# Chlumsky/msdfgen

Hardware: AMD Instinct MI355X
Metric: MSDF glyphs/sec (64x64, fp32) (higher is better)
Workload: dtype f64

## Files before the change

### msdfgen_amd/csrc/msdf_capi.hip

```cpp

#include <hip/hip_runtime.h>

#include <algorithm>
#include <atomic>
#include <chrono>
#include <condition_variable>
#include <cmath>
#include <cstdarg>
#include <cstdio>
#include <cstdlib>
#include <cstring>
#include <deque>
#include <functional>
#include <memory>
#include <mutex>
#include <string>
#include <thread>
#include <vector>

#include <sched.h>

#include "msdf_classplan.hpp"
#include "msdf_hostplan.hpp"
#include "msdf_kernels.hpp"
// ... 881 lines not shown
        return rc;
    ScopedTimer timer(stream, 1, !paramsOnly);
    if (cfg.ec_stage_limit != 0) {
        if (paramsOnly)
            return MSDFHIP_OK;
        const unsigned cap = GRES ? slowGrid : 16384u;
        const unsigned slowBlocks = (unsigned) ((allTexels+WAVE-1)/WAVE < cap ? (allTexels+WAVE-1)/WAVE : cap);
        hipLaunchKernelGGL((k_ec_slow<N, OVERLAP, GRES>), dim3(slowBlocks), dim3(WAVE), slowLds, stream, viewOf(b), dGlyphs, w, h, src, out, stencil, cfg,
                           (const EcCandidate *) NULL, 0u, 0, gres, gresStride);
        HIPCHK(hipGetLastError());
        return MSDFHIP_OK;
    }
    const unsigned seg = ecSegment((size_t) w*h);
    const size_t cap = deferredRecords(b->nGlyphs, (size_t) w*h, b->nEdges);
    EcCandidate *deferred = NULL;
    rc = ensureDeferred(b, cap, &deferred);
    if (rc != MSDFHIP_OK)
        return rc;
    const int slotCapWanted = tuning().querySlotCap, lpcContoursWanted = tuning().queryLpcContours;
    int slotCap = b->maxEdges < slotCapWanted ? (b->maxEdges > 0 ? b->maxEdges : 1) : slotCapWanted;
    bool wideSlots = false;
    if (b->nGlyphs < 256 && !tuning().hasQueryLds) {
        const int wide = b->maxEdges < 1024 ? (b->maxEdges > 0 ? b->maxEdges : 1) : 1024;
        const int wideMerged = b->maxContours < wide ? (b->maxContours > 0 ? b->maxContours : 1) : wide;
        if ((size_t) b->maxContours*sizeof(double)+(size_t) (wide+wideMerged)*sizeof(PBSlot) <= (size_t) 64*1024 && wide > slotCap)
            slotCap = wide, wideSlots = true;
    }
    EcQueryPolicy lpcMaxContours;
    lpcMaxContours.lpcMaxContours = b->maxContours < lpcContoursWanted ? b->maxContours : lpcContoursWanted;
    lpcMaxContours.lpcEdgeCost = tuning().qpEdgeCost, lpcMaxContours.lpcMaxEdges = tuning().qpMaxEdges, lpcMaxContours.lpcMinCount = tuning().qpMinCount;
    lpcMaxContours.wideMaxEdges = tuning().qpWideMaxEdges, lpcMaxContours.wideLoad = tuning().qpWideLoad, lpcMaxContours.wideMeanCount = tuning().qpWideMeanCount;
    lpcMaxContours.gridSteps = tuning().queryGridSteps;
    const size_t resLanes = OVERLAP ? (size_t) (lpcMaxContours.lpcMaxContours > 0 ? lpcMaxContours.lpcMaxContours : 1)*WAVE*sizeof(double) : 0;
    const int slotOffset = OVERLAP ? (b->maxContours > 0 ? b->maxContours : 1) : 0;
    const int mergedCap = b->maxContours < slotCap ? (b->maxContours > 0 ? b->maxContours : 1) : slotCap;
    const size_t coopLds = (size_t) slotOffset*sizeof(double)+(size_t) (slotCap+mergedCap)*sizeof(PBSlot);
    const size_t queryLds = resLanes > coopLds ? resLanes : coopLds;
    const size_t fastLds = ecFastLdsBytes(b->maxEdges, N);
    if (GRES && queryLds > (size_t) gLdsLimit.load() && fastLds <= (size_t) gLdsLimit.load()) {
        if (paramsOnly)
            return MSDFHIP_OK;
        hipLaunchKernelGGL((k_ec_slow<N, OVERLAP, GRES>), dim3(slowGrid), dim3(WAVE), slowLds, stream, viewOf(b), dGlyphs, w, h, src, out, stencil, cfg,
                           (const EcCandidate *) NULL, 0u, 0, gres, gresStride);
        HIPCHK(hipGetLastError());
        countRoute(MSDFHIP_ROUTE_EC_SLOW_ALL);
        return MSDFHIP_OK;
    }
    if (fastLds > (size_t) gLdsLimit.load() || queryLds > (size_t) gLdsLimit.load())
        return fail(MSDFHIP_ERR_TOO_COMPLEX, "a glyph has %d contours / %d edges: the error-correction pass needs %zu B of LDS per wavefront, device limit is %d B",
                    b->maxContours, b->maxEdges, fastLds > queryLds ? fastLds : queryLds, gLdsLimit.load());
    rc = setLds(k_ec_query<N, OVERLAP>, queryLds);
    if (rc != MSDFHIP_OK)
        return rc;
    rc = setLds(k_ec_fast<N>, fastLds);
    if (rc != MSDFHIP_OK)
        return rc;
    int *offsets = reinterpret_cast<int *>(deferred+candidateRecords(b->nGlyphs, (size_t) w*h));
    int *corners = reinterpret_cast<int *>(deferred+candidateRecords(b->nGlyphs, (size_t) w*h)+offsetRecords(b->nGlyphs));
    const size_t wanted = allTexels/512;
    unsigned queryBlocks = (unsigned) (wanted < 64 ? 64 : wanted > 8192 ? 8192 : wanted);
    const bool staticDeal = tuning().queryStatic != 0;
    if (staticDeal) {
        const unsigned resident = queryResidentBlocks<N, OVERLAP>(b->device, queryLds);
        if (resident && queryBlocks > resident)
            queryBlocks = resident;
    }
    if (!call.ecParamsQueued)
        hipLaunchKernelGGL(k_ec_params, dim3((unsigned) b->nGlyphs), dim3(WAVE), 0, stream, b->work.ecParams.ptr, viewOf(b), dGlyphs, cfg,
                           reinterpret_cast<unsigned *>(deferred), corners, offsets+ecSizesAt(b->nGlyphs));
    const int *ecOrder = NULL;
    rc = ensureEcOrder(b, &ecOrder, stream);
    if (rc != MSDFHIP_OK)
        return rc;
    if (paramsOnly) {
        HIPCHK(hipGetLastError());
        call.ecParamsQueued = true;
        return MSDFHIP_OK;
    }
    hipLaunchKernelGGL((k_ec_fast<N>), dim3(blocks), dim3(WAVE), fastLds, stream, viewOf(b), dGlyphs, w, h, tilesX, tiles, src, out, stencil, cfg,
                       (const EcGlyphParams *) b->work.ecParams.ptr, deferred, seg, b->maxEdges, (const int *) corners);
    hipLaunchKernelGGL(k_ec_scan, dim3(1), dim3(1024), 0, stream, b->nGlyphs, reinterpret_cast<const unsigned *>(deferred), seg, offsets, lpcMaxContours, ecOrder);
    hipLaunchKernelGGL((k_ec_query<N, OVERLAP>), dim3(queryBlocks), dim3(WAVE), queryLds, stream, b->nGlyphs, b->dGlyphContourOffsets, b->dContourOffsets,
                       (const EdgeRec *) viewOf(b).recs, viewOf(b).windings, dGlyphs, w, h, src, out, stencil, cfg,
                       (const EcGlyphParams *) b->work.ecParams.ptr, (const EcCandidate *) deferred, seg, (const int *) offsets, offsets+2*(size_t) b->nGlyphs+2, tuning().queryBatch, slotCap, slotOffset, lpcMaxContours,
                       call.overflowOut, ecOrder, staticDeal ? (tuning().queryStatic == 2 ? 5 : 1) : 0);
    if (call.overflowOut)
        call.overflowMirrored = true;
    else
        hipLaunchKernelGGL((k_ec_slow<N, OVERLAP, GRES>), dim3(slowGrid), dim3(WAVE), slowLds, stream, viewOf(b), dGlyphs, w, h, src, out, stencil, cfg,
                           (const EcCandidate *) deferred, seg, 1, gres, gresStride);
    HIPCHK(hipGetLastError());
    countRoute(ecOrder ? MSDFHIP_ROUTE_EC_QUERY_HEAVIEST : MSDFHIP_ROUTE_EC_QUERY_BATCH);
    if (wideSlots)
        countRoute(MSDFHIP_ROUTE_EC_WIDE_SLOTS);
    return MSDFHIP_OK;
}

template <int N>
int dispatchEc(const MsdfHipBatch *b, const MsdfHipGlyph *dGlyphs, int w, int h, const float *src, float *out, uint8_t *stencil,
               const MsdfHipConfig &cfg, hipStream_t stream, GenerateCall &call, bool paramsOnly) {
    if (!cfg.overlap_support)
        return launchEc<N, false, false>(b, dGlyphs, w, h, src, out, stencil, cfg, stream, call, paramsOnly);
    const bool globalRes = (size_t) b->maxContours*WAVE*sizeof(double) > 96*1024;
    return globalRes ? launchEc<N, true, true>(b, dGlyphs, w, h, src, out, stencil, cfg, stream, call, paramsOnly)
                     : launchEc<N, true, false>(b, dGlyphs, w, h, src, out, stencil, cfg, stream, call, paramsOnly);
}

int checkConfig(const MsdfHipConfig *cfg) {
    if (!cfg)
        return fail(MSDFHIP_ERR_INVALID, "cfg is NULL");
    if (cfg->ec_mode < 0 || cfg->ec_mode > 3 || cfg->ec_distance_check < 0 || cfg->ec_distance_check > 2 || cfg->ec_stage_limit < 0 || cfg->ec_stage_limit > 4)
        return fail(MSDFHIP_ERR_INVALID, "bad error-correction config (mode %d, distance check %d, stage limit %d)", cfg->ec_mode, cfg->ec_distance_check, cfg->ec_stage_limit);
    return MSDFHIP_OK;
}

int ensureScratch(const MsdfHipBatch *b, size_t floats, float **out) {
    std::lock_guard<std::mutex> lock(b->work.mutex);
    HIPCHK(b->work.scratch.ensure(floats));
    *out = b->work.scratch.ptr;
    return MSDFHIP_OK;
}

int runCorrection(const MsdfHipBatch *b, int channels, int w, int h, const MsdfHipGlyph *dGlyphs, const float *src, float *out, uint8_t *stencil,
                  const MsdfHipConfig &cfg, hipStream_t stream, GenerateCall &call, bool paramsOnly) {
    return channels == 3 ? dispatchEc<3>(b, dGlyphs, w, h, src, out, stencil, cfg, stream, call, paramsOnly)
                         : dispatchEc<4>(b, dGlyphs, w, h, src, out, stencil, cfg, stream, call, paramsOnly);
}

int prepareAhead(const MsdfHipBatch *b, int mode, int w, int h, const MsdfHipGlyph *dGlyphs, const MsdfHipConfig *cfg, hipStream_t stream, GenerateCall &call) {
    if (b->nGlyphs == 0 || w == 0 || h == 0)
        return MSDFHIP_OK;
    const int nch = channelsOf(mode);
    const LaunchShape shape = launchShape(b, w, h, nch, false);
// ... 2970 lines not shown
```

### msdfgen_amd/csrc/msdf_ec_fast.hpp

```cpp
#pragma once

#include "msdf_ec.hpp"

namespace msdfhip {

enum { EC_DEFER = 0x80 };

MSDF_HD bool ecHasBasePass(const EcParams &p) { return p.distanceCheck == EC_DO_NOT_CHECK || (p.distanceCheck == EC_CHECK_AT_EDGE && p.mode != EC_MODE_EDGE_ONLY); }
MSDF_HD bool ecHasShapePass(const EcParams &p) { return p.distanceCheck == EC_ALWAYS_CHECK || p.distanceCheck == EC_CHECK_AT_EDGE; }

struct FastCtx {
    double span;
    bool p1;
    bool pShape;
    bool basePass, shapePass;
};

MSDF_HD int rangeTest2(const FastCtx &c, double at, double bt, double xt, float am, float bm, float xm) {
    const bool inversion = (am > .5f && bm > .5f && xm <= .5f) || (am < .5f && bm < .5f && xm >= .5f);
    const bool outside = medianf(am, bm, xm) != xm;
    const bool candBase = c.basePass && (inversion || (!c.p1 && outside));
    const bool candShape = c.shapePass && (inversion || (!c.pShape && outside));
    if (!(candBase || candShape))
        return 0;
    const double axSpan = (xt-at)*c.span, bxSpan = (bt-xt)*c.span;
    const int f = (xm >= am-axSpan && xm <= am+axSpan && xm >= bm-bxSpan && xm <= bm+bxSpan) ? 1 : 3;
    return (candBase ? f : 0)|(candShape ? f<<2 : 0);
}

MSDF_HD int judge(int flags) {
    if (flags&2)
        return 1;
    const int fs = flags>>2;
    if (fs&1)
        return (fs&2) ? 1 : 2;
    return 0;
}

MSDF_HD bool quadraticMayHaveRootInRange(double a, double b, double c) {
    if (a == 0 || fabs(b) > 1e12*fabs(a))
        return true;
    const double lo = .005, hi = .995;
    const double mag = fabs(a)+fabs(b)+fabs(c);
    const double eps = 1e-9*mag;
    const double flo = (a*lo+b)*lo+c, fhi = (a*hi+b)*hi+c;
    if (!(flo > eps && fhi > eps) && !(flo < -eps && fhi < -eps))
        return true;
    const double s = flo > 0 ? 1. : -1.;
    const double as = a*s, bs = b*s, cs = c*s;
    if (as <= 0)
        return false;
    if (!(-bs > 2*as*lo*(1-1e-9) && -bs < 2*as*hi*(1+1e-9)))
        return false;
    return !(4*as*cs-bs*bs > 1e-9*mag*mag);
}

MSDF_HD bool bernsteinMayHaveRoot(float dA, float dBC, float dD) {
    const float m = fmaxf(fmaxf(fabsf(dA), fabsf(dBC)), fabsf(dD));
    const float eps = 1e-5f*m;
    const float h = .5f*dBC;
    return !((dA > eps && h > eps && dD > eps) || (dA < -eps && h < -eps && dD < -eps));
}

MSDF_HD bool edgeBetweenTexelsChannelFast(const float *a, const float *b, int channel) {
    const double n = a[channel]-.5;
    const double d = a[channel]-b[channel];
    if (!((n > 0 && d > 0 && n < d) || (n < 0 && d < 0 && n > d)))
        return false;
    const double t = n/d;
    if (t > 0 && t < 1) {
        float c[3] = { mixf(a[0], b[0], t), mixf(a[1], b[1], t), mixf(a[2], b[2], t) };
        return medianf(c[0], c[1], c[2]) == c[channel];
    }
    return false;
}

MSDF_HD int edgeBetweenTexelsFast(const float *a, const float *b) {
    return 1*(int) edgeBetweenTexelsChannelFast(a, b, 0)+2*(int) edgeBetweenTexelsChannelFast(a, b, 1)+4*(int) edgeBetweenTexelsChannelFast(a, b, 2);
}

template <class Sink>
MSDF_HD int diagonalPairFast(const FastCtx &cx, float am, float dm, const float *a, const float *l, const float *q,
                             float dA, float dBC, float dD, float l0, float q0, float l1, float q1, Sink &sink) {
    const double qa = dD-dBC+dA, qb = dBC-dA-dA, qc = dA;
    if (!quadraticMayHaveRootInRange(qa, qb, qc))
        return 0;
    double t[2];
    const int solutions = solveQuadratic(t, qa, qb, qc);
    int verdict = 0;
    for (int i = 0; i < solutions; ++i) {
        if (t[i] > MSDF_ARTIFACT_T_EPSILON && t[i] < 1-MSDF_ARTIFACT_T_EPSILON) {
            const float xm = interpolatedMedianQuad(a, l, q, t[i]);
            int rangeFlags = rangeTest2(cx, 0, 1, t[i], am, dm, xm);
            const double tEx0 = -.5*l0/q0, tEx1 = -.5*l1/q1;
            if (tEx0 > 0 && tEx0 < 1) {
                double tEnd0 = 0, tEnd1 = 1;
                float em0 = am, em1 = dm;
                const float ex = interpolatedMedianQuad(a, l, q, tEx0);
                if (tEx0 > t[i])
                    tEnd1 = tEx0, em1 = ex;
                else
                    tEnd0 = tEx0, em0 = ex;
                rangeFlags |= rangeTest2(cx, tEnd0, tEnd1, t[i], em0, em1, xm);
            }
            if (tEx1 > 0 && tEx1 < 1) {
                double tEnd0 = 0, tEnd1 = 1;
                float em0 = am, em1 = dm;
                const float ex = interpolatedMedianQuad(a, l, q, tEx1);
                if (tEx1 > t[i])
                    tEnd1 = tEx1, em1 = ex;
                else
                    tEnd0 = tEx1, em0 = ex;
                rangeFlags |= rangeTest2(cx, tEnd0, tEnd1, t[i], em0, em1, xm);
            }
            const int v = judge(rangeFlags);
            if (v&2)
                sink(t[i]);
            verdict |= v;
            if (verdict&1)
                return verdict;
        }
    }
    return verdict;
}

struct Neighbourhood {
    float v[3][3][3];
    float dev[3][3];
    unsigned valid;
};

MSDF_HD float ecTexelDeviation(const float *t) { return fabsf(medianf(t[0], t[1], t[2])-.5f); }

MSDF_HD void loadNeighbourhood(Neighbourhood &nb, const SdfView &sdf, int x, int yn) {
    nb.valid = 0;
    MSDF_UNROLL
    for (int dy = -1; dy <= 1; ++dy) {
        MSDF_UNROLL
        for (int dx = -1; dx <= 1; ++dx) {
            const int nx = x+dx, ny = yn+dy;
            const bool in = nx >= 0 && ny >= 0 && nx < sdf.w && ny < sdf.h;
            const float *t = sdf.native(in ? nx : x, in ? ny : yn);
            nb.v[dy+1][dx+1][0] = t[0], nb.v[dy+1][dx+1][1] = t[1], nb.v[dy+1][dx+1][2] = t[2];
            nb.dev[dy+1][dx+1] = ecTexelDeviation(t);
            if (in)
                nb.valid |= 1u<<((dy+1)*3+(dx+1));
        }
    }
}

template <class Emit>
MSDF_HD void texelProtectPairs(const Neighbourhood &nb, const EcParams &p, Emit &emit) {
    const float sdev = nb.dev[1][1];
    MSDF_UNROLL
    for (int dy = -1; dy <= 1; ++dy) {
        MSDF_UNROLL
        for (int dx = -1; dx <= 1; ++dx) {
            if (!dx && !dy)
                continue;
            if (!(nb.valid&(1u<<((dy+1)*3+(dx+1)))))
                continue;
            const float radius = dy == 0 ? p.radiusH : dx == 0 ? p.radiusV : p.radiusD;
            const float odev = nb.dev[dy+1][dx+1];
            const bool selfIsA = dy > 0 || (dy == 0 && dx > 0);
            const float sum = selfIsA ? sdev+odev : odev+sdev;
            if (sum < radius)
                emit((dy+1)*3+(dx+1));
        }
    }
}

MSDF_HD bool evaluateProtectPair(const float *self, const float *other, int m) {
// ... 14 lines not shown
    for (int i = 0; i < items.n; ++i)
        if (evaluateProtectPair(nb.v[1][1], nb.v[items.m[i]/3][items.m[i]%3], items.m[i]))
            return true;
    return false;
}

MSDF_HD int ecNeighbourDx(int k) { return k < 4 ? (k == 0 ? -1 : k == 2 ? 1 : 0) : ((k&1) ? 1 : -1); }
MSDF_HD int ecNeighbourDy(int k) { return k < 4 ? (k == 1 ? -1 : k == 3 ? 1 : 0) : ((k&2) ? 1 : -1); }

template <class Emit>
MSDF_HD void texelCandidatePairs(const Neighbourhood &nb, Emit &emit) {
    const float *c = nb.v[1][1];
    const float cdev = nb.dev[1][1];
    MSDF_UNROLL
    for (int k = 0; k < 4; ++k) {
        const int dx = k == 0 ? -1 : k == 2 ? 1 : 0, dy = k == 1 ? -1 : k == 3 ? 1 : 0;
        if (!(nb.valid&(1u<<((dy+1)*3+(dx+1)))))
            continue;
        const float *b = nb.v[dy+1][dx+1];
        if (!(cdev >= nb.dev[dy+1][dx+1]))
            continue;
        MSDF_UNROLL
        for (int j = 0; j < 3; ++j) {
            const int i0 = j, i1 = j == 2 ? 0 : j+1;
            const float dA = c[i1]-c[i0], dB = b[i1]-b[i0];
            if ((dA > 0 && dB < 0) || (dA < 0 && dB > 0))
                emit(k, j);
        }
    }
    MSDF_UNROLL
    for (int k = 4; k < 8; ++k) {
        const int dx = (k&1) ? 1 : -1, dy = (k&2) ? 1 : -1;
        if (!(nb.valid&(1u<<((dy+1)*3+(dx+1)))))
            continue;
        const float *d = nb.v[dy+1][dx+1];
        if (!(cdev >= nb.dev[dy+1][dx+1]))
            continue;
        const float *b = nb.v[1][dx+1], *cc = nb.v[dy+1][1];
        MSDF_UNROLL
        for (int j = 0; j < 3; ++j) {
            const int i0 = j, i1 = j == 2 ? 0 : j+1;
            const float dA = c[i1]-c[i0], dBC = b[i1]-b[i0]+cc[i1]-cc[i0], dD = d[i1]-d[i0];
            if (dA == 0 && dBC == 0 && dD == 0)
                continue;
            if (bernsteinMayHaveRoot(dA, dBC, dD))
                emit(k, j);
        }
    }
}

MSDF_HD float pick3(const float *v, int i) { return i == 0 ? v[0] : i == 1 ? v[1] : v[2]; }

template <class Sink>
MSDF_HD int evaluatePair(const float *c, const float *n, const float *hb, const float *vc, const EcParams &p, bool p1, int flip, int k, int j, Sink &sink) {
    FastCtx cx;
    cx.basePass = ecHasBasePass(p);
    cx.shapePass = ecHasShapePass(p);
    cx.p1 = p1;
    cx.pShape = (p.distanceCheck == EC_CHECK_AT_EDGE) ? true : p1;
    const int dx = ecNeighbourDx(k), dy = ecNeighbourDy(k);
    const int i0 = j, i1 = j == 2 ? 0 : j+1;
    const float cm = medianf(c[0], c[1], c[2]), nm = medianf(n[0], n[1], n[2]);
    if (k < 4) {
        cx.span = dy == 0 ? p.hSpan : p.vSpan;
        const float dA = pick3(c, i1)-pick3(c, i0), dB = pick3(n, i1)-pick3(n, i0);
        const double t = (double) dA/(dA-dB);
        if (t > MSDF_ARTIFACT_T_EPSILON && t < 1-MSDF_ARTIFACT_T_EPSILON) {
            const float xm = interpolatedMedianLin(c, n, t);
            const int v = judge(rangeTest2(cx, 0, 1, t, cm, nm, xm));
            if (v&2)
                sink(t, dx, flip ? -dy : dy);
            return v;
        }
        return 0;
    }
    cx.span = p.dSpan;
    const float *a = c, *b = hb, *cc = vc, *d = n;
    const float abc[3] = { a[0]-b[0]-cc[0], a[1]-b[1]-cc[1], a[2]-b[2]-cc[2] };
    const float l[3] = { -a[0]-abc[0], -a[1]-abc[1], -a[2]-abc[2] };
    const float q[3] = { d[0]+abc[0], d[1]+abc[1], d[2]+abc[2] };
    const float a3[3] = { a[0], a[1], a[2] };
    struct DirSink {
        Sink &sink;
        int dx, dy;
        MSDF_HD void operator()(double t) { sink(t, dx, dy); }
    } dirSink = { sink, dx, flip ? -dy : dy };
    const float dA = pick3(a, i1)-pick3(a, i0), dBC = pick3(b, i1)-pick3(b, i0)+pick3(cc, i1)-pick3(cc, i0), dD = pick3(d, i1)-pick3(d, i0);
    return diagonalPairFast(cx, cm, nm, a3, l, q, dA, dBC, dD, pick3(l, i0), pick3(q, i0), pick3(l, i1), pick3(q, i1), dirSink);
}

template <class Sink>
MSDF_HD int texelFindFast(const Neighbourhood &nb, const EcParams &p, bool p1, int flip, Sink &sink) {
    struct Items {
        unsigned char k[24], j[24];
        int n;
        MSDF_HD void operator()(int kk, int jj) { k[n] = (unsigned char) kk, j[n] = (unsigned char) jj; ++n; }
    } items;
    items.n = 0;
    texelCandidatePairs(nb, items);
    int verdict = 0;
    for (int i = 0; i < items.n; ++i) {
        const int k = items.k[i], dx = ecNeighbourDx(k), dy = ecNeighbourDy(k);
        verdict |= evaluatePair(nb.v[1][1], nb.v[dy+1][dx+1], nb.v[1][dx+1], nb.v[dy+1][1], p, p1, flip, k, items.j[i], sink);
    }
    return verdict;
}

template <class Sink>
MSDF_HD int ecTexelFast(const SdfView &sdf, const EcParams &p, const int *corners, int nCorners, int x, int yn, Sink &sink) {
    const int ys = sdf.flip ? sdf.h-1-yn : yn;
    Neighbourhood nb;
    loadNeighbourhood(nb, sdf, x, yn);
    int st = 0;
    if (p.mode == EC_MODE_EDGE_PRIORITY) {
        for (int i = 0; i < nCorners; ++i) {
            const int l = corners[2*i], b = corners[2*i+1];
            if ((x == l || x == l+1) && (ys == b || ys == b+1)) {
                st |= EC_PROTECTED;
                break;
            }
        }
        if (!(st&EC_PROTECTED) && protectedByEdgesNb(nb, p))
            st |= EC_PROTECTED;
    } else if (p.mode == EC_MODE_EDGE_ONLY)
        st |= EC_PROTECTED;
    const int verdict = texelFindFast(nb, p, (st&EC_PROTECTED) != 0, sdf.flip, sink);
    if (ecHasBasePass(p) && p.distanceCheck == EC_CHECK_AT_EDGE)
        st |= EC_PROTECTED;
    if (verdict&1)
        st |= EC_ERROR;
    else if (verdict&2)
        st |= EC_DEFER;
    return st;
}

template <class Query>
MSDF_HD bool ecEvaluateCandidate(const SdfView &sdf, const EcParams &p, int x, int ys, double t, int dx, int dy, const Query &query) {
    const float *msd = sdf.shape(x, ys);
    const V2 tVector = t*mk(dx, dy);
    float oldMSD[3], newMSD[3];
    interpolate3(oldMSD, sdf, mk(x+.5, ys+.5)+tVector);
    const double aWeight = (1-fabs(tVector.x))*(1-fabs(tVector.y));
    const float aPSD = medianf(msd[0], msd[1], msd[2]);
    newMSD[0] = (float) (oldMSD[0]+aWeight*(aPSD-msd[0]));
    newMSD[1] = (float) (oldMSD[1]+aWeight*(aPSD-msd[1]));
    newMSD[2] = (float) (oldMSD[2]+aWeight*(aPSD-msd[2]));
    const float oldPSD = medianf(oldMSD[0], oldMSD[1], oldMSD[2]);
    const float newPSD = medianf(newMSD[0], newMSD[1], newMSD[2]);
    const V2 q = unproject(p.t, mk(x+.5, ys+.5))+mk(tVector.x*p.texelX, tVector.y*p.texelY);
    const float refPSD = mapDistance(p.t, query(q));
    return p.minImproveRatio*fabsf(newPSD-refPSD) < (double) fabsf(oldPSD-refPSD);
}

}
```

### msdfgen_amd/csrc/msdf_kernels.hpp

```cpp
#pragma once

#include <hip/hip_runtime.h>
#include "msdf_device.hpp"
#include "msdf_prep.hpp"
#include "msdf_ec.hpp"
#include "msdf_ec_fast.hpp"
#include "msdf_cull.hpp"
#include "msdf_scanline.hpp"
#include "msdf_shapeprep.hpp"
#include "msdf_frame.hpp"
#include "../../include/msdfgen_hip.h"

namespace msdfhip {

#ifndef MSDF_DISTANCE_WAVES_PER_SIMD
#define MSDF_DISTANCE_WAVES_PER_SIMD 4
#endif
constexpr int TILE = 8;
constexpr int WAVE = 64;
constexpr int REC_DOUBLES = sizeof(EdgeRec)/sizeof(double);

struct BatchView {
    int nGlyphs;
    const int32_t *glyphContourOffsets;
// ... 954 lines not shown
__device__ __forceinline__ void ecParamsBody(EcGlyphParams *out, const BatchView &batch, const MsdfHipGlyph *glyphs, const MsdfHipConfig &cfg, unsigned *candidateHeader,
                                             int *corners, int *sizes, const int g, const int lane) {
    if (candidateHeader && lane == 0) {
        candidateHeader[1+g] = 0;
        if (g == 0)
            candidateHeader[0] = 0;
    }
    EcParams p;
    p.t = loadXform(glyphs[g]);
    p.minDeviationRatio = cfg.min_deviation_ratio;
    p.minImproveRatio = cfg.min_improve_ratio;
    ecDerive(p);
    const int c0 = batch.glyphContourOffsets[g], C = batch.glyphContourOffsets[g+1]-c0;
    const int e0 = batch.contourOffsets[c0], nE = batch.contourOffsets[c0+C]-e0;
    int nCorners = 0;
    if (cfg.ec_mode == EC_MODE_EDGE_PRIORITY && corners) {
        const EdgeRec *rec = batch.recs+e0;
        for (int base = 0; base < nE; base += WAVE) {
            const int e = base+lane;
            const bool corner = e < nE && (rec[e].flags&REC_CORNER);
            const unsigned long long mask = __ballot(corner);
            if (corner) {
                const V2 pp = project(p.t, ld(rec[e].p0));
                const int slot = e0+nCorners+__popcll(mask&((1ull<<lane)-1ull));
                corners[2*slot] = (int) floor(pp.x-.5);
                corners[2*slot+1] = (int) floor(pp.y-.5);
            }
            nCorners += __popcll(mask);
        }
    }
    if (lane == 0) {
        EcGlyphParams o;
        o.hSpan = p.hSpan, o.vSpan = p.vSpan, o.dSpan = p.dSpan, o.texelX = p.texelX, o.texelY = p.texelY;
        o.radiusH = p.radiusH, o.radiusV = p.radiusV, o.radiusD = p.radiusD, o.cornerBegin = e0, o.nCorners = nCorners, o.pad = 0;
        out[g] = o;
        if (sizes)
            sizes[2*g] = nE, sizes[2*g+1] = C;
    }
}
__global__ void __launch_bounds__(WAVE)
k_ec_params(EcGlyphParams *out, BatchView batch, const MsdfHipGlyph *glyphs, MsdfHipConfig cfg, unsigned *candidateHeader, int *corners, int *sizes) {
    ecParamsBody(out, batch, glyphs, cfg, candidateHeader, corners, sizes, (int) blockIdx.x, (int) threadIdx.x);
}

#ifndef MSDF_EC_FAST_WAVES_PER_SIMD
#define MSDF_EC_FAST_WAVES_PER_SIMD 7
#endif
enum { EC_HALO = TILE+2, EC_QUEUE_CAP = WAVE*24, EC_PROTECT_QUEUE_CAP = WAVE*8 };
__host__ __device__ inline size_t ecFastLdsBytes(int maxEdges, int n) {
    return (size_t) EC_HALO*EC_HALO*n*sizeof(float)+(WAVE+4)*sizeof(int)
           +(EC_QUEUE_CAP+EC_PROTECT_QUEUE_CAP)*sizeof(unsigned short);
}

template <int N>
__device__ __forceinline__ void ecFastBody(const BatchView &batch, const MsdfHipGlyph *glyphs, int width, int height, int tilesX, int tilesPerGlyph,
          const float *src, float *out, uint8_t *stencilOut, const MsdfHipConfig &cfg, const EcGlyphParams *glyphParams, EcCandidate *cands, unsigned seg,
          int maxEdges, const int *corners, const unsigned blockId, int *smemFast, const int sinkSlots = 0, const int sinkSlot = 0) {
    const GlyphWork wk = decodeItem(blockId, batch.nGlyphs, tilesPerGlyph);
    if (!wk.valid)
        return;
    float *halo = reinterpret_cast<float *>(smemFast);
    int *verdictLds = reinterpret_cast<int *>(halo+EC_HALO*EC_HALO*N);
    int *itemCount = verdictLds+WAVE;
    unsigned short *queue = reinterpret_cast<unsigned short *>(itemCount+4);
    unsigned short *protectQueue = queue+EC_QUEUE_CAP;
    float *devLds = reinterpret_cast<float *>(queue+EC_QUEUE_CAP)-EC_HALO*EC_HALO;
    static_assert((EC_QUEUE_CAP*sizeof(unsigned short))%sizeof(float) == 0 && EC_QUEUE_CAP*sizeof(unsigned short) >= EC_HALO*EC_HALO*sizeof(float), "devLds overlays the queue's tail");
    const int lane = threadIdx.x;
    const MsdfHipGlyph gd = glyphs[wk.g];
    EcParams p;
    p.t = loadXform(gd);
    p.minDeviationRatio = cfg.min_deviation_ratio;
    p.minImproveRatio = cfg.min_improve_ratio;
    p.mode = cfg.ec_mode, p.distanceCheck = cfg.ec_distance_check, p.overlap = cfg.overlap_support, p.stageLimit = 0;
    const EcGlyphParams gp = glyphParams[wk.g];
    p.hSpan = gp.hSpan, p.vSpan = gp.vSpan, p.dSpan = gp.dSpan, p.texelX = gp.texelX, p.texelY = gp.texelY;
    p.radiusH = gp.radiusH, p.radiusV = gp.radiusV, p.radiusD = gp.radiusD;
    const int tx = wk.tile%tilesX, ty = wk.tile/tilesX;

    const int lxT = lane&(TILE-1), lyT = lane>>3;
    const int xT = tx*TILE+lxT, ysT = gd.flip ? height-1-(ty*TILE+lyT) : ty*TILE+lyT;
    bool cornerTexel = false;
    if (p.mode == EC_MODE_EDGE_PRIORITY) {
        const int x0 = tx*TILE, x1 = tx*TILE+TILE-1;
        const int ya = gd.flip ? height-1-(ty*TILE+TILE-1) : ty*TILE, yb = gd.flip ? height-1-ty*TILE : ty*TILE+TILE-1;
        const int *list = corners+2*(size_t) gp.cornerBegin;
        for (int base = 0; base < gp.nCorners; base += WAVE) {
            const int k = base+lane;
            int l = 0, b = 0;
            bool near = false;
            if (k < gp.nCorners) {
                l = list[2*k], b = list[2*k+1];
                near = l+1 >= x0 && l <= x1 && b+1 >= ya && b <= yb;
            }
            for (unsigned long long mask = __ballot(near); mask; mask &= mask-1) {
                const int src = __ffsll((long long) mask)-1;
                const int cl = __builtin_amdgcn_readlane(l, src), cb = __builtin_amdgcn_readlane(b, src);
                cornerTexel = cornerTexel || ((xT == cl || xT == cl+1) && (ysT == cb || ysT == cb+1));
            }
        }
    }

    const float *field = src+(size_t) wk.g*height*width*N;
    for (int idx = lane; idx < EC_HALO*EC_HALO; idx += WAVE) {
        const int hx = tx*TILE+idx%EC_HALO-1, hy = ty*TILE+idx/EC_HALO-1;
        if (hx >= 0 && hy >= 0 && hx < width && hy < height) {
            const float *t = field+((size_t) hy*width+hx)*N;
            float tv[N];
            for (int ch = 0; ch < N; ++ch)
                tv[ch] = t[ch], halo[idx*N+ch] = tv[ch];
            devLds[idx] = ecTexelDeviation(tv);
        }
    }
    if (lane < 2)
        itemCount[lane] = 0;
    waveSync();

    const int lx = lane&(TILE-1), ly = lane>>3;
    const int x = tx*TILE+lx, yn = ty*TILE+ly;
    const bool inside = x < width && yn < height;
    int st = 0;
    const bool classify = inside;
    Neighbourhood nb;
    nb.valid = 0;
    if (classify) {
        MSDF_UNROLL
        for (int dy = -1; dy <= 1; ++dy) {
            MSDF_UNROLL
            for (int dx = -1; dx <= 1; ++dx) {
                const int nx = x+dx, ny = yn+dy;
                const bool in = nx >= 0 && ny >= 0 && nx < width && ny < height;
                const float *t = halo+((ly+1+(in ? dy : 0))*EC_HALO+lx+1+(in ? dx : 0))*N;
                nb.v[dy+1][dx+1][0] = t[0], nb.v[dy+1][dx+1][1] = t[1], nb.v[dy+1][dx+1][2] = t[2];
                nb.dev[dy+1][dx+1] = devLds[(ly+1+(in ? dy : 0))*EC_HALO+lx+1+(in ? dx : 0)];
                if (in)
                    nb.valid |= 1u<<((dy+1)*3+(dx+1));
            }
        }
    }
    waveSync();
    if (classify) {
        if (p.mode == EC_MODE_EDGE_PRIORITY) {
            if (cornerTexel)
                st |= EC_PROTECTED;
            if (!(st&EC_PROTECTED)) {
                struct PushProtect {
                    unsigned short *queue;
                    int *count;
                    int lane;
                    __device__ void operator()(int m) { queue[atomicAdd(count, 1)] = (unsigned short) (lane|m<<6); }
                } pushProtect = { protectQueue, itemCount+1, lane };
                texelProtectPairs(nb, p, pushProtect);
            }
        } else if (p.mode == EC_MODE_EDGE_ONLY)
            st |= EC_PROTECTED;
        struct Push {
            unsigned short *queue;
            int *count;
            int lane;
            __device__ void operator()(int k, int j) { queue[atomicAdd(count, 1)] = (unsigned short) (lane|k<<6|j<<9); }
        } push = { queue, itemCount, lane };
        texelCandidatePairs(nb, push);
    }
    verdictLds[lane] = (st&EC_PROTECTED) ? 0x100 : 0;
    waveSync();

    const int nProtect = itemCount[1];
    for (int base = 0; base < nProtect; base += WAVE) {
        const int it = base+lane;
        if (it >= nProtect)
            continue;
        const unsigned item = protectQueue[it];
        const int s = item&63, m = item>>6;
        const int sx = s&(TILE-1), sy = s>>3;
        const float *self = halo+((sy+1)*EC_HALO+sx+1)*N, *other = halo+((sy+m/3)*EC_HALO+sx+m%3)*N;
        if (evaluateProtectPair(self, other, m))
            atomicOr(&verdictLds[s], 0x100);
    }
    waveSync();

    const int nItems = itemCount[0];
    for (int base = 0; base < nItems; base += WAVE) {
        const int it = base+lane;
        if (it >= nItems)
            continue;
        const unsigned item = queue[it];
        const int s = item&63, k = (item>>6)&7, jp = item>>9;
        const int sx = s&(TILE-1), sy = s>>3;
        const int dx = ecNeighbourDx(k), dy = ecNeighbourDy(k);
        const float *c = halo+((sy+1)*EC_HALO+sx+1)*N, *n = halo+((sy+1+dy)*EC_HALO+sx+1+dx)*N;
        const float *hb = halo+((sy+1)*EC_HALO+sx+1+dx)*N, *vc = halo+((sy+1+dy)*EC_HALO+sx+1)*N;
        CandidateSink sink;
        sink.header = reinterpret_cast<unsigned *>(cands);
        sink.segment = sinkSlots > 0 ? cands+ecHeaderRecords(sinkSlots)+(size_t) sinkSlot*seg : cands+ecHeaderRecords(batch.nGlyphs)+(size_t) wk.g*seg;
        sink.seg = seg, sink.g = sinkSlots > 0 ? sinkSlot : wk.g;
        sink.texel = (unsigned) (((size_t) wk.g*height+ty*TILE+sy)*width+tx*TILE+sx);
        const int v = evaluatePair(c, n, hb, vc, p, (verdictLds[s]&0x100) != 0, gd.flip, k, jp, sink);
        if (v)
            atomicOr(&verdictLds[s], v);
    }
    waveSync();

    if (!inside)
        return;
    const int verdict = verdictLds[lane];
    if ((verdict&0x100) || (ecHasBasePass(p) && p.distanceCheck == EC_CHECK_AT_EDGE))
        st |= EC_PROTECTED;
    if (verdict&1)
        st |= EC_ERROR;
    const size_t texel = ((size_t) wk.g*height+yn)*width+x;
    const float *in = halo+((ly+1)*EC_HALO+lx+1)*N;
    float v[N];
    for (int i = 0; i < N; ++i)
        v[i] = in[i];
    if (st&EC_ERROR) {
        const float m = medianf(v[0], v[1], v[2]);
        v[0] = m, v[1] = m, v[2] = m;
    }
    float *px = out+gd.out_offset+(ptrdiff_t) gd.row_stride*yn+(ptrdiff_t) N*x;
    for (int i = 0; i < N; ++i)
        px[i] = v[i];
    if (stencilOut)
        stencilOut[stencilIndex(texel, yn, width, height, cfg.stencil_y_down)] = (uint8_t) st;
}
template <int N>
__global__ void __launch_bounds__(WAVE, MSDF_EC_FAST_WAVES_PER_SIMD)
k_ec_fast(BatchView batch, const MsdfHipGlyph *glyphs, int width, int height, int tilesX, int tilesPerGlyph,
          const float *src, float *out, uint8_t *stencilOut, MsdfHipConfig cfg, const EcGlyphParams *glyphParams, EcCandidate *cands, unsigned seg,
          int maxEdges, const int *corners) {
    extern __shared__ int smemFast[];
    ecFastBody<N>(batch, glyphs, width, height, tilesX, tilesPerGlyph, src, out, stencilOut, cfg, glyphParams, cands, seg, maxEdges, corners, blockIdx.x, smemFast);
}

struct EcQueryPolicy { int lpcMaxContours, lpcEdgeCost, lpcMaxEdges, lpcMinCount, wideMaxEdges; float wideLoad, wideMeanCount; int gridSteps; };
MSDF_HD int ecQueryGridSlices(unsigned count, int nE, int C, EcQueryPolicy q) {
    if (q.gridSteps <= 0 || C > q.lpcMaxContours || count == 0)
        return 0;
    int J = 1;
    while (J < (int) count && J < WAVE)
        J <<= 1;
    int S = WAVE/J, need = 1;
    while (need*q.gridSteps < nE && need < WAVE)
        need <<= 1;
    if (need > S)
        S = need;
    return S >= 2 && S <= WAVE/2 ? S : 0;
}
MSDF_HD bool ecQueryLanePerCandidate(unsigned count, int nE, int C, EcQueryPolicy q) {
    if (C > q.lpcMaxContours)
        return false;
    if ((nE > q.lpcMaxEdges && (int) count < q.lpcMinCount))
        return false;
    const long long coop = (long long) count*(340ll*((nE+WAVE-1)/WAVE)+10ll*nE+1000ll);
    const long long lpc = (long long) ((count+WAVE-1)/WAVE)*((long long) q.lpcEdgeCost*nE+1000ll);
    return lpc < coop;
}
MSDF_HD int ecQueryItems(unsigned count, unsigned seg, int nE, int C, EcQueryPolicy lpcMaxContours) {
    if (count > seg)
        return 0;
    const int S = ecQueryGridSlices(count, nE, C, lpcMaxContours);
    if (S)
        return (int) ((count+WAVE/S-1)/(WAVE/S));
    return ecQueryLanePerCandidate(count, nE, C, lpcMaxContours) ? (int) ((count+WAVE-1)/WAVE) : (int) count;
}
MSDF_HD bool ecQueryListedFirst(unsigned count, int nE, int C, EcQueryPolicy q) {
    return ecQueryGridSlices(count, nE, C, q) != 0 || ecQueryLanePerCandidate(count, nE, C, q) || (q.gridSteps > 0 && nE > WAVE);
}

MSDF_HD size_t ecQueuesAt(int nGlyphs) { return 2*((size_t) nGlyphs+1)+2+2*(size_t) nGlyphs; }
MSDF_HD size_t ecOffsetInts(int nGlyphs) { return ecQueuesAt(nGlyphs)+8*16; }
MSDF_HD size_t ecSizesAt(int nGlyphs) { return 2*((size_t) nGlyphs+1)+2; }

__global__ void __launch_bounds__(1024)
k_ec_scan(int nGlyphs, const unsigned *__restrict__ header, unsigned seg, int *__restrict__ offsets, EcQueryPolicy lpcMaxContours, const int *__restrict__ order) {
    __shared__ int waveTotals[2][16];
    __shared__ float waveLoad[16], waveCount[16];
    enum { PER = 8 };
    const int t = threadIdx.x, lane = t&(WAVE-1), wave = t/WAVE;
    const int *sizes = offsets+ecSizesAt(nGlyphs);
    float mine = 0, mineCount = 0;
    for (int base = 0; base < nGlyphs; base += 1024*PER) {
        unsigned count[PER];
        int nE[PER];
        MSDF_UNROLL
// ... 816 lines not shown
```

Measured before the change: 1.718 million.

## Defer edge-priority protection checks in error-correction fast pass until artifacts need them

In edge-priority mode with check-at-edge distance checking, the fast error-correction kernel no longer computes corner and edge protection for every texel up front. It first evaluates artifact pairs assuming protection, flags texels whose verdict depends on protection, and runs the corner scan and protect queue only for those. Held candidates are then re-evaluated for protected texels. This avoids protection work on most texels, at the cost of extra passes, more branching and a second kernel template instantiation.

```diff
diff --git a/msdfgen_amd/csrc/msdf_capi.hip b/msdfgen_amd/csrc/msdf_capi.hip
--- a/msdfgen_amd/csrc/msdf_capi.hip
+++ b/msdfgen_amd/csrc/msdf_capi.hip
@@ -957,7 +957,8 @@
     rc = setLds(k_ec_query<N, OVERLAP>, queryLds);
     if (rc != MSDFHIP_OK)
         return rc;
-    rc = setLds(k_ec_fast<N>, fastLds);
+    const bool lazyProtect = cfg.ec_mode == EC_MODE_EDGE_PRIORITY && cfg.ec_distance_check == EC_CHECK_AT_EDGE;
+    rc = lazyProtect ? setLds(k_ec_fast<N, true>, fastLds) : setLds(k_ec_fast<N, false>, fastLds);
     if (rc != MSDFHIP_OK)
         return rc;
     int *offsets = reinterpret_cast<int *>(deferred+candidateRecords(b->nGlyphs, (size_t) w*h));
@@ -982,8 +983,12 @@
         call.ecParamsQueued = true;
         return MSDFHIP_OK;
     }
-    hipLaunchKernelGGL((k_ec_fast<N>), dim3(blocks), dim3(WAVE), fastLds, stream, viewOf(b), dGlyphs, w, h, tilesX, tiles, src, out, stencil, cfg,
-                       (const EcGlyphParams *) b->work.ecParams.ptr, deferred, seg, b->maxEdges, (const int *) corners);
+    if (lazyProtect)
+        hipLaunchKernelGGL((k_ec_fast<N, true>), dim3(blocks), dim3(WAVE), fastLds, stream, viewOf(b), dGlyphs, w, h, tilesX, tiles, src, out, stencil, cfg,
+                           (const EcGlyphParams *) b->work.ecParams.ptr, deferred, seg, b->maxEdges, (const int *) corners);
+    else
+        hipLaunchKernelGGL((k_ec_fast<N, false>), dim3(blocks), dim3(WAVE), fastLds, stream, viewOf(b), dGlyphs, w, h, tilesX, tiles, src, out, stencil, cfg,
+                           (const EcGlyphParams *) b->work.ecParams.ptr, deferred, seg, b->maxEdges, (const int *) corners);
     hipLaunchKernelGGL(k_ec_scan, dim3(1), dim3(1024), 0, stream, b->nGlyphs, reinterpret_cast<const unsigned *>(deferred), seg, offsets, lpcMaxContours, ecOrder);
     hipLaunchKernelGGL((k_ec_query<N, OVERLAP>), dim3(queryBlocks), dim3(WAVE), queryLds, stream, b->nGlyphs, b->dGlyphContourOffsets, b->dContourOffsets,
                        (const EdgeRec *) viewOf(b).recs, viewOf(b).windings, dGlyphs, w, h, src, out, stencil, cfg,
diff --git a/msdfgen_amd/csrc/msdf_ec_fast.hpp b/msdfgen_amd/csrc/msdf_ec_fast.hpp
--- a/msdfgen_amd/csrc/msdf_ec_fast.hpp
+++ b/msdfgen_amd/csrc/msdf_ec_fast.hpp
@@ -5,15 +5,23 @@
 namespace msdfhip {
 
 enum { EC_DEFER = 0x80 };
+
+enum { EC_V_ERROR = 1,
+       EC_V_CHECK = 2,
+       EC_V_COND = 4,
+       EC_V_HELD = 8 };
+enum { EC_ORDER_EAGER = 0, EC_ORDER_LAZY = 1, EC_ORDER_LAZY_HELD = 2 };
 
 MSDF_HD bool ecHasBasePass(const EcParams &p) { return p.distanceCheck == EC_DO_NOT_CHECK || (p.distanceCheck == EC_CHECK_AT_EDGE && p.mode != EC_MODE_EDGE_ONLY); }
 MSDF_HD bool ecHasShapePass(const EcParams &p) { return p.distanceCheck == EC_ALWAYS_CHECK || p.distanceCheck == EC_CHECK_AT_EDGE; }
+MSDF_HD bool ecLazyProtect(const EcParams &p) { return p.mode == EC_MODE_EDGE_PRIORITY && p.distanceCheck == EC_CHECK_AT_EDGE; }
 
 struct FastCtx {
     double span;
     bool p1;
     bool pShape;
     bool basePass, shapePass;
+    int order;
 };
 
 MSDF_HD int rangeTest2(const FastCtx &c, double at, double bt, double xt, float am, float bm, float xm) {
@@ -21,20 +29,22 @@
     const bool outside = medianf(am, bm, xm) != xm;
     const bool candBase = c.basePass && (inversion || (!c.p1 && outside));
     const bool candShape = c.shapePass && (inversion || (!c.pShape && outside));
-    if (!(candBase || candShape))
+    const bool candCond = c.order != EC_ORDER_EAGER && !inversion && outside;
+    if (!(candBase || candShape || candCond))
         return 0;
     const double axSpan = (xt-at)*c.span, bxSpan = (bt-xt)*c.span;
     const int f = (xm >= am-axSpan && xm <= am+axSpan && xm >= bm-bxSpan && xm <= bm+bxSpan) ? 1 : 3;
-    return (candBase ? f : 0)|(candShape ? f<<2 : 0);
+    return (candBase ? f : 0)|(candShape ? f<<2 : 0)|(candCond && f == 3 ? 16 : 0);
 }
 
 MSDF_HD int judge(int flags) {
+    const int cond = (flags&16) ? EC_V_COND : 0;
     if (flags&2)
-        return 1;
-    const int fs = flags>>2;
+        return EC_V_ERROR|cond;
+    const int fs = (flags>>2)&3;
     if (fs&1)
-        return (fs&2) ? 1 : 2;
-    return 0;
+        return ((fs&2) ? EC_V_ERROR : EC_V_CHECK)|cond;
+    return cond;
 }
 
 MSDF_HD bool quadraticMayHaveRootInRange(double a, double b, double c) {
@@ -114,10 +124,15 @@
                 rangeFlags |= rangeTest2(cx, tEnd0, tEnd1, t[i], em0, em1, xm);
             }
             const int v = judge(rangeFlags);
-            if (v&2)
-                sink(t[i]);
             verdict |= v;
-            if (verdict&1)
+            if (v&EC_V_CHECK) {
+                const bool held = (verdict&EC_V_COND) != 0;
+                if (held)
+                    verdict |= EC_V_HELD;
+                if (held == (cx.order == EC_ORDER_LAZY_HELD))
+                    sink(t[i]);
+            }
+            if (verdict&EC_V_ERROR)
                 return verdict;
         }
     }
@@ -238,23 +253,27 @@
 MSDF_HD float pick3(const float *v, int i) { return i == 0 ? v[0] : i == 1 ? v[1] : v[2]; }
 
 template <class Sink>
-MSDF_HD int evaluatePair(const float *c, const float *n, const float *hb, const float *vc, const EcParams &p, bool p1, int flip, int k, int j, Sink &sink) {
+MSDF_HD int evaluatePair(const float *c, const float *n, const float *hb, const float *vc, const EcParams &p, bool p1, int flip, int k, int j, Sink &sink,
+                         int order = EC_ORDER_EAGER) {
     FastCtx cx;
     cx.basePass = ecHasBasePass(p);
     cx.shapePass = ecHasShapePass(p);
-    cx.p1 = p1;
-    cx.pShape = (p.distanceCheck == EC_CHECK_AT_EDGE) ? true : p1;
+    cx.order = order;
+    cx.p1 = order != EC_ORDER_EAGER || p1;
+    cx.pShape = (p.distanceCheck == EC_CHECK_AT_EDGE) ? true : cx.p1;
     const int dx = ecNeighbourDx(k), dy = ecNeighbourDy(k);
     const int i0 = j, i1 = j == 2 ? 0 : j+1;
     const float cm = medianf(c[0], c[1], c[2]), nm = medianf(n[0], n[1], n[2]);
     if (k < 4) {
+        if (order == EC_ORDER_LAZY_HELD)
+            return 0;
         cx.span = dy == 0 ? p.hSpan : p.vSpan;
         const float dA = pick3(c, i1)-pick3(c, i0), dB = pick3(n, i1)-pick3(n, i0);
         const double t = (double) dA/(dA-dB);
         if (t > MSDF_ARTIFACT_T_EPSILON && t < 1-MSDF_ARTIFACT_T_EPSILON) {
             const float xm = interpolatedMedianLin(c, n, t);
             const int v = judge(rangeTest2(cx, 0, 1, t, cm, nm, xm));
-            if (v&2)
+            if (v&EC_V_CHECK)
                 sink(t, dx, flip ? -dy : dy);
             return v;
         }
@@ -276,7 +295,7 @@
 }
 
 template <class Sink>
-MSDF_HD int texelFindFast(const Neighbourhood &nb, const EcParams &p, bool p1, int flip, Sink &sink) {
+MSDF_HD int texelFindFast(const Neighbourhood &nb, const EcParams &p, bool p1, int flip, Sink &sink, int order = EC_ORDER_EAGER) {
     struct Items {
         unsigned char k[24], j[24];
         int n;
@@ -287,35 +306,49 @@
     int verdict = 0;
     for (int i = 0; i < items.n; ++i) {
         const int k = items.k[i], dx = ecNeighbourDx(k), dy = ecNeighbourDy(k);
-        verdict |= evaluatePair(nb.v[1][1], nb.v[dy+1][dx+1], nb.v[1][dx+1], nb.v[dy+1][1], p, p1, flip, k, items.j[i], sink);
+        verdict |= evaluatePair(nb.v[1][1], nb.v[dy+1][dx+1], nb.v[1][dx+1], nb.v[dy+1][1], p, p1, flip, k, items.j[i], sink, order);
     }
     return verdict;
 }
 
+MSDF_HD bool protectedByCornerList(const int *corners, int nCorners, int x, int ys) {
+    for (int i = 0; i < nCorners; ++i) {
+        const int l = corners[2*i], b = corners[2*i+1];
+        if ((x == l || x == l+1) && (ys == b || ys == b+1))
+            return true;
+    }
+    return false;
+}
+
+MSDF_HD bool ecNeedsProtection(int verdict) { return ((verdict&EC_V_COND) && !(verdict&EC_V_ERROR)) || (verdict&EC_V_HELD); }
+
 template <class Sink>
-MSDF_HD int ecTexelFast(const SdfView &sdf, const EcParams &p, const int *corners, int nCorners, int x, int yn, Sink &sink) {
+MSDF_HD int ecTexelFast(const SdfView &sdf, const EcParams &p, const int *corners, int nCorners, int x, int yn, Sink &sink, bool allowLazy = true) {
     const int ys = sdf.flip ? sdf.h-1-yn : yn;
     Neighbourhood nb;
     loadNeighbourhood(nb, sdf, x, yn);
-    int st = 0;
-    if (p.mode == EC_MODE_EDGE_PRIORITY) {
-        for (int i = 0; i < nCorners; ++i) {
-            const int l = corners[2*i], b = corners[2*i+1];
-            if ((x == l || x == l+1) && (ys == b || ys == b+1)) {
+    int st = 0, verdict;
+    if (allowLazy && ecLazyProtect(p)) {
+        verdict = texelFindFast(nb, p, true, sdf.flip, sink, EC_ORDER_LAZY);
+        if (ecNeedsProtection(verdict)) {
+            if (!(protectedByCornerList(corners, nCorners, x, ys) || protectedByEdgesNb(nb, p)))
+                verdict |= EC_V_ERROR;
+            else if (verdict&EC_V_HELD)
+                texelFindFast(nb, p, true, sdf.flip, sink, EC_ORDER_LAZY_HELD);
+        }
+    } else {
+        if (p.mode == EC_MODE_EDGE_PRIORITY) {
+            if (protectedByCornerList(corners, nCorners, x, ys) || protectedByEdgesNb(nb, p))
                 st |= EC_PROTECTED;
-                break;
-            }
-        }
-        if (!(st&EC_PROTECTED) && protectedByEdgesNb(nb, p))
+        } else if (p.mode == EC_MODE_EDGE_ONLY)
             st |= EC_PROTECTED;
-    } else if (p.mode == EC_MODE_EDGE_ONLY)
-        st |= EC_PROTECTED;
-    const int verdict = texelFindFast(nb, p, (st&EC_PROTECTED) != 0, sdf.flip, sink);
+        verdict = texelFindFast(nb, p, (st&EC_PROTECTED) != 0, sdf.flip, sink);
+    }
     if (ecHasBasePass(p) && p.distanceCheck == EC_CHECK_AT_EDGE)
         st |= EC_PROTECTED;
-    if (verdict&1)
+    if (verdict&EC_V_ERROR)
         st |= EC_ERROR;
-    else if (verdict&2)
+    else if (verdict&EC_V_CHECK)
         st |= EC_DEFER;
     return st;
 }
diff --git a/msdfgen_amd/csrc/msdf_kernels.hpp b/msdfgen_amd/csrc/msdf_kernels.hpp
--- a/msdfgen_amd/csrc/msdf_kernels.hpp
+++ b/msdfgen_amd/csrc/msdf_kernels.hpp
@@ -1030,7 +1030,52 @@
            +(EC_QUEUE_CAP+EC_PROTECT_QUEUE_CAP)*sizeof(unsigned short);
 }
 
+__device__ __forceinline__ bool ecTileCornerTexel(const int *list, int nCorners, int tx, int ty, int height, int flip, int lane) {
+    const int lxT = lane&(TILE-1), lyT = lane>>3;
+    const int xT = tx*TILE+lxT, ysT = flip ? height-1-(ty*TILE+lyT) : ty*TILE+lyT;
+    const int x0 = tx*TILE, x1 = tx*TILE+TILE-1;
+    const int ya = flip ? height-1-(ty*TILE+TILE-1) : ty*TILE, yb = flip ? height-1-ty*TILE : ty*TILE+TILE-1;
+    bool cornerTexel = false;
+    for (int base = 0; base < nCorners; base += WAVE) {
+        const int k = base+lane;
+        int l = 0, b = 0;
+        bool near = false;
+        if (k < nCorners) {
+            l = list[2*k], b = list[2*k+1];
+            near = l+1 >= x0 && l <= x1 && b+1 >= ya && b <= yb;
+        }
+        for (unsigned long long mask = __ballot(near); mask; mask &= mask-1) {
+            const int src = __ffsll((long long) mask)-1;
+            const int cl = __builtin_amdgcn_readlane(l, src), cb = __builtin_amdgcn_readlane(b, src);
+            cornerTexel = cornerTexel || ((xT == cl || xT == cl+1) && (ysT == cb || ysT == cb+1));
+        }
+    }
+    return cornerTexel;
+}
+
 template <int N>
+__device__ __forceinline__ void ecRunProtectQueue(const float *halo, const unsigned short *protectQueue, int nProtect, int *verdictLds, int lane) {
+    for (int base = 0; base < nProtect; base += WAVE) {
+        const int it = base+lane;
+        if (it >= nProtect)
+            continue;
+        const unsigned item = protectQueue[it];
+        const int s = item&63, m = item>>6;
+        const int sx = s&(TILE-1), sy = s>>3;
+        const float *self = halo+((sy+1)*EC_HALO+sx+1)*N, *other = halo+((sy+m/3)*EC_HALO+sx+m%3)*N;
+        if (evaluateProtectPair(self, other, m))
+            atomicOr(&verdictLds[s], 0x100);
+    }
+}
+
+struct EcPushProtect {
+    unsigned short *queue;
+    int *count;
+    int lane;
+    __device__ void operator()(int m) { queue[atomicAdd(count, 1)] = (unsigned short) (lane|m<<6); }
+};
+
+template <int N, int ORDER = -1>
 __device__ __forceinline__ void ecFastBody(const BatchView &batch, const MsdfHipGlyph *glyphs, int width, int height, int tilesX, int tilesPerGlyph,
           const float *src, float *out, uint8_t *stencilOut, const MsdfHipConfig &cfg, const EcGlyphParams *glyphParams, EcCandidate *cands, unsigned seg,
           int maxEdges, const int *corners, const unsigned blockId, int *smemFast, const int sinkSlots = 0, const int sinkSlot = 0) {
@@ -1056,28 +1101,10 @@
     p.radiusH = gp.radiusH, p.radiusV = gp.radiusV, p.radiusD = gp.radiusD;
     const int tx = wk.tile%tilesX, ty = wk.tile/tilesX;
 
-    const int lxT = lane&(TILE-1), lyT = lane>>3;
-    const int xT = tx*TILE+lxT, ysT = gd.flip ? height-1-(ty*TILE+lyT) : ty*TILE+lyT;
+    const bool lazy = ORDER < 0 ? ecLazyProtect(p) : ORDER != 0;
     bool cornerTexel = false;
-    if (p.mode == EC_MODE_EDGE_PRIORITY) {
-        const int x0 = tx*TILE, x1 = tx*TILE+TILE-1;
-        const int ya = gd.flip ? height-1-(ty*TILE+TILE-1) : ty*TILE, yb = gd.flip ? height-1-ty*TILE : ty*TILE+TILE-1;
-        const int *list = corners+2*(size_t) gp.cornerBegin;
-        for (int base = 0; base < gp.nCorners; base += WAVE) {
-            const int k = base+lane;
-            int l = 0, b = 0;
-            bool near = false;
-            if (k < gp.nCorners) {
-                l = list[2*k], b = list[2*k+1];
-                near = l+1 >= x0 && l <= x1 && b+1 >= ya && b <= yb;
-            }
-            for (unsigned long long mask = __ballot(near); mask; mask &= mask-1) {
-                const int src = __ffsll((long long) mask)-1;
-                const int cl = __builtin_amdgcn_readlane(l, src), cb = __builtin_amdgcn_readlane(b, src);
-                cornerTexel = cornerTexel || ((xT == cl || xT == cl+1) && (ysT == cb || ysT == cb+1));
-            }
-        }
-    }
+    if (p.mode == EC_MODE_EDGE_PRIORITY && !lazy)
+        cornerTexel = ecTileCornerTexel(corners+2*(size_t) gp.cornerBegin, gp.nCorners, tx, ty, height, gd.flip, lane);
 
     const float *field = src+(size_t) wk.g*height*width*N;
     for (int idx = lane; idx < EC_HALO*EC_HALO; idx += WAVE) {
@@ -1118,16 +1145,11 @@
     }
     waveSync();
     if (classify) {
-        if (p.mode == EC_MODE_EDGE_PRIORITY) {
+        if (p.mode == EC_MODE_EDGE_PRIORITY && !lazy) {
             if (cornerTexel)
                 st |= EC_PROTECTED;
             if (!(st&EC_PROTECTED)) {
-                struct PushProtect {
-                    unsigned short *queue;
-                    int *count;
-                    int lane;
-                    __device__ void operator()(int m) { queue[atomicAdd(count, 1)] = (unsigned short) (lane|m<<6); }
-                } pushProtect = { protectQueue, itemCount+1, lane };
+                EcPushProtect pushProtect = { protectQueue, itemCount+1, lane };
                 texelProtectPairs(nb, p, pushProtect);
             }
         } else if (p.mode == EC_MODE_EDGE_ONLY)
@@ -1143,48 +1165,89 @@
     verdictLds[lane] = (st&EC_PROTECTED) ? 0x100 : 0;
     waveSync();
 
-    const int nProtect = itemCount[1];
-    for (int base = 0; base < nProtect; base += WAVE) {
-        const int it = base+lane;
-        if (it >= nProtect)
-            continue;
-        const unsigned item = protectQueue[it];
-        const int s = item&63, m = item>>6;
-        const int sx = s&(TILE-1), sy = s>>3;
-        const float *self = halo+((sy+1)*EC_HALO+sx+1)*N, *other = halo+((sy+m/3)*EC_HALO+sx+m%3)*N;
-        if (evaluateProtectPair(self, other, m))
-            atomicOr(&verdictLds[s], 0x100);
-    }
+    if (!lazy) {
+        ecRunProtectQueue<N>(halo, protectQueue, itemCount[1], verdictLds, lane);
+        waveSync();
+    }
+
+    const int nItems = itemCount[0];
+    const auto runItems = [&](const int order) {
+        for (int base = 0; base < nItems; base += WAVE) {
+            const int it = base+lane;
+            if (it >= nItems)
+                continue;
+            const unsigned item = queue[it];
+            const int s = item&63, k = (item>>6)&7, jp = item>>9;
+            const int word = verdictLds[s];
+            if (order == EC_ORDER_LAZY_HELD && (word&(0x100|EC_V_HELD)) != (0x100|EC_V_HELD))
+                continue;
+            const int sx = s&(TILE-1), sy = s>>3;
+            const int dx = ecNeighbourDx(k), dy = ecNeighbourDy(k);
+            const float *c = halo+((sy+1)*EC_HALO+sx+1)*N, *n = halo+((sy+1+dy)*EC_HALO+sx+1+dx)*N;
+            const float *hb = halo+((sy+1)*EC_HALO+sx+1+dx)*N, *vc = halo+((sy+1+dy)*EC_HALO+sx+1)*N;
+            CandidateSink sink;
+            sink.header = reinterpret_cast<unsigned *>(cands);
+            sink.segment = sinkSlots > 0 ? cands+ecHeaderRecords(sinkSlots)+(size_t) sinkSlot*seg : cands+ecHeaderRecords(batch.nGlyphs)+(size_t) wk.g*seg;
+            sink.seg = seg, sink.g = sinkSlots > 0 ? sinkSlot : wk.g;
+            sink.texel = (unsigned) (((size_t) wk.g*height+ty*TILE+sy)*width+tx*TILE+sx);
+            const int v = evaluatePair(c, n, hb, vc, p, (word&0x100) != 0, gd.flip, k, jp, sink, order);
+            if (v && order != EC_ORDER_LAZY_HELD)
+                atomicOr(&verdictLds[s], v);
+        }
+    };
+    runItems(lazy ? EC_ORDER_LAZY : EC_ORDER_EAGER);
     waveSync();
 
-    const int nItems = itemCount[0];
-    for (int base = 0; base < nItems; base += WAVE) {
-        const int it = base+lane;
-        if (it >= nItems)
-            continue;
-        const unsigned item = queue[it];
-        const int s = item&63, k = (item>>6)&7, jp = item>>9;
-        const int sx = s&(TILE-1), sy = s>>3;
-        const int dx = ecNeighbourDx(k), dy = ecNeighbourDy(k);
-        const float *c = halo+((sy+1)*EC_HALO+sx+1)*N, *n = halo+((sy+1+dy)*EC_HALO+sx+1+dx)*N;
-        const float *hb = halo+((sy+1)*EC_HALO+sx+1+dx)*N, *vc = halo+((sy+1+dy)*EC_HALO+sx+1)*N;
-        CandidateSink sink;
-        sink.header = reinterpret_cast<unsigned *>(cands);
-        sink.segment = sinkSlots > 0 ? cands+ecHeaderRecords(sinkSlots)+(size_t) sinkSlot*seg : cands+ecHeaderRecords(batch.nGlyphs)+(size_t) wk.g*seg;
-        sink.seg = seg, sink.g = sinkSlots > 0 ? sinkSlot : wk.g;
-        sink.texel = (unsigned) (((size_t) wk.g*height+ty*TILE+sy)*width+tx*TILE+sx);
-        const int v = evaluatePair(c, n, hb, vc, p, (verdictLds[s]&0x100) != 0, gd.flip, k, jp, sink);
-        if (v)
-            atomicOr(&verdictLds[s], v);
-    }
-    waveSync();
+    const bool need = lazy && inside && ecNeedsProtection(verdictLds[lane]);
+    if (__ballot(need)) {
+        __asm__ volatile("" ::: "memory");
+        const EcGlyphParams gl = glyphParams[wk.g];
+        EcParams pr = p;
+        pr.radiusH = gl.radiusH, pr.radiusV = gl.radiusV, pr.radiusD = gl.radiusD;
+        cornerTexel = ecTileCornerTexel(corners+2*(size_t) gl.cornerBegin, gl.nCorners, tx, ty, height, gd.flip, lane);
+        if (need) {
+            if (cornerTexel)
+                verdictLds[lane] |= 0x100;
+            else {
+                Neighbourhood nd;
+                nd.valid = 0;
+                MSDF_UNROLL
+                for (int dy = -1; dy <= 1; ++dy) {
+                    MSDF_UNROLL
+                    for (int dx = -1; dx <= 1; ++dx) {
+                        const int nx = x+dx, ny = yn+dy;
+                        const bool in = nx >= 0 && ny >= 0 && nx < width && ny < height;
+                        nd.dev[dy+1][dx+1] = ecTexelDeviation(halo+((ly+1+(in ? dy : 0))*EC_HALO+lx+1+(in ? dx : 0))*N);
+                        if (in)
+                            nd.valid |= 1u<<((dy+1)*3+(dx+1));
+                    }
+                }
+                EcPushProtect pushProtect = { protectQueue, itemCount+1, lane };
+                texelProtectPairs(nd, pr, pushProtect);
+            }
+        }
+        waveSync();
+        ecRunProtectQueue<N>(halo, protectQueue, itemCount[1], verdictLds, lane);
+        waveSync();
+        bool revisit = false;
+        if (need) {
+            const int word = verdictLds[lane];
+            if (!(word&0x100))
+                verdictLds[lane] = word|EC_V_ERROR;
+            revisit = (word&0x100) && (word&EC_V_HELD);
+        }
+        if (__ballot(revisit)) {
+            waveSync();
+            runItems(EC_ORDER_LAZY_HELD);
+        }
+    }
 
     if (!inside)
         return;
     const int verdict = verdictLds[lane];
     if ((verdict&0x100) || (ecHasBasePass(p) && p.distanceCheck == EC_CHECK_AT_EDGE))
         st |= EC_PROTECTED;
-    if (verdict&1)
+    if (verdict&EC_V_ERROR)
         st |= EC_ERROR;
     const size_t texel = ((size_t) wk.g*height+yn)*width+x;
     const float *in = halo+((ly+1)*EC_HALO+lx+1)*N;
@@ -1201,13 +1264,13 @@
     if (stencilOut)
         stencilOut[stencilIndex(texel, yn, width, height, cfg.stencil_y_down)] = (uint8_t) st;
 }
-template <int N>
+template <int N, bool LAZY>
 __global__ void __launch_bounds__(WAVE, MSDF_EC_FAST_WAVES_PER_SIMD)
 k_ec_fast(BatchView batch, const MsdfHipGlyph *glyphs, int width, int height, int tilesX, int tilesPerGlyph,
           const float *src, float *out, uint8_t *stencilOut, MsdfHipConfig cfg, const EcGlyphParams *glyphParams, EcCandidate *cands, unsigned seg,
           int maxEdges, const int *corners) {
     extern __shared__ int smemFast[];
-    ecFastBody<N>(batch, glyphs, width, height, tilesX, tilesPerGlyph, src, out, stencilOut, cfg, glyphParams, cands, seg, maxEdges, corners, blockIdx.x, smemFast);
+    ecFastBody<N, LAZY ? 1 : 0>(batch, glyphs, width, height, tilesX, tilesPerGlyph, src, out, stencilOut, cfg, glyphParams, cands, seg, maxEdges, corners, blockIdx.x, smemFast);
 }
 
 struct EcQueryPolicy { int lpcMaxContours, lpcEdgeCost, lpcMaxEdges, lpcMinCount, wideMaxEdges; float wideLoad, wideMeanCount; int gridSteps; };
```

Result: faster. 1.820 million (median of 6 runs) (+5.9%).
